# factoryofthesun/distraytracer

Measured on NVIDIA B200. Metric: samples_per_s_1080p_64spp, higher is better.
Workload: dtype f64

## Files before the change

distraytracer_b200/csrc/drt_api.cu:

```cuda
#include <cuda_runtime.h>

#include <algorithm>
#include <cmath>
#include <cstdio>
#include <cstdlib>
#include <cstring>
#include <string>
#include <vector>

#include "../../include/drt.h"
#include "drt_box.cuh"
#include "drt_launch.h"
#include "drt_bvh_order.h"
#include "drt_mesh.h"
#include "drt_skeleton.h"

using namespace drt;

namespace {

thread_local std::string g_err;
int fail(int code, const std::string& m) { g_err = m; return code; }

#define CK(call)                                                                                   \
// ... 569 lines not shown

template <typename R>
void fillParams(Params<R>& P, const drt_scene* s, const DevScene<R>& ds, const drt_settings& st, const CameraD& c, const drt_tile& tile) {
  memset(&P, 0, sizeof(P));
  P.eye = cv<R>(c.eye); P.X = cv<R>(c.X); P.Y = cv<R>(c.Y); P.Z = cv<R>(c.Z);
  for (int i = 0; i < 12; i++) { P.mcam[i] = (R)c.mcam[i]; P.new_mcam[i] = (R)c.new_mcam[i]; P.cloud_mcam[i] = (R)c.cloud_mcam[i]; }
  P.t = c.t; P.b = c.b; P.r = c.r; P.l = c.l;
  P.near_plane = st.near_plane; P.focal_length = st.focal_length; P.aperture = st.aperture;
  P.xRes = st.xRes; P.yRes = st.yRes;
  P.n = (int)sqrt((double)st.antialias_samples);
  P.spp = P.n * P.n;
  P.antialias_samples = st.antialias_samples;
  P.brdf_samples = st.brdf_samples; P.blur_samples = st.blur_samples; P.frame_range = st.frame_range; P.max_depth = st.max_depth;
  P.reflect = st.reflect; P.nogloss = st.nogloss; P.perlin_cloud = st.perlin_cloud; P.cloud_only = st.cloud_only;
  P.frame = st.frame; P.frame_prism = st.frame_prism; P.frame_blur = st.frame_blur; P.frame_cloud = st.frame_cloud;
  P.move_per_frame = st.move_per_frame; P.accel_t = st.accel_t; P.refr_air = st.refr_air; P.refr_glass = st.refr_glass;
  P.phong = st.phong; P.seed = st.seed; P.blur_mode = st.blur_mode;
  P.swept_cull = (st.blur_mode == DRT_BLUR_VELOCITY && st.frame_range <= DRT_SWEPT_FRAMES) ? 1 : 0;
  P.sun = cv<R>(normalized(V(st.sundir)));
  f3(P.sun_outer, st.sun_outer); f3(P.sun_inner, st.sun_inner); f3(P.sun_core, st.sun_core);
  f3(P.bluesky, st.bluesky); f3(P.redsky, st.redsky);
  P.saturation = st.saturation; P.clouddist = st.clouddist; P.cloudhoff = st.cloudhoff;
  P.x0 = tile.x0; P.y0 = tile.y0; P.w = tile.width; P.h = tile.height;
  P.geoms = ds.geoms; P.n_geoms = ds.n_geoms; P.gbounds = ds.gbounds; P.geom_tree = ds.geom_tree >= 0 ? ds.gbounds + ds.geom_tree : nullptr; P.nodes = ds.nodes; P.n_nodes = ds.n_nodes; P.prims = ds.prims; P.lights = ds.lights; P.n_lights = ds.n_lights;
  P.tex = s->d_tex; P.texdims = s->d_texdims;
  if (s->has_mesh) {
    P.mesh_nodes = s->mesh.nodes; P.n_mesh_tris = s->mesh.n_tris; P.mesh_prim = (int)s->prims.size();
    if constexpr (sizeof(R) == 8) P.mesh_tris = s->mesh.tris_f64; else P.mesh_tris = s->mesh.tris_f32;
    P.mesh_mat = s->mesh.mat_ids;
    const drt_prim& m0 = s->mesh_materials[0];
    P.mesh_vel = mk<R>((R)m0.velocity[0], (R)m0.velocity[1], (R)m0.velocity[2]);
  } else P.mesh_vel = mk<R>(R(0), R(0), R(0));
}

int ensureScratch(drt_scene* s, size_t n_samples, size_t n_corners, size_t n_out) {
  CK(s->samples.reserve(n_samples * sizeof(float4)));
  CK(s->need.reserve(n_corners));
  CK(s->bg.reserve(n_corners * sizeof(float4)));
  CK(s->out_u8.reserve(n_out));
  CK(s->out_f32.reserve(n_out * sizeof(float)));
  CK(s->counts.reserve(sizeof(Counts)));
  CK(s->batch_counter.reserve(sizeof(unsigned long long)));
  if (!s->overflow) { CK(s->overflow.reserve(sizeof(int))); CK(cudaMemsetAsync(s->overflow, 0, sizeof(int), s->stream)); }
  return DRT_OK;
}

long long maxChunkSamples() {
// ... 623 lines not shown
```

distraytracer_b200/csrc/drt_device.cuh:

```cuda
#pragma once
#include <cuda_runtime.h>
#include <stdint.h>
#include <float.h>
#include <math.h>
#include <utility>

#include "drt_rng.cuh"

#define DRT_PI 3.14159265358979323846
#define DRT_NODE_STACK 64

namespace drt {

template <typename R> struct Vec { R x, y, z; };

template <typename R> __host__ __device__ inline Vec<R> mk(R x, R y, R z) { Vec<R> v; v.x = x; v.y = y; v.z = z; return v; }
template <typename R> __host__ __device__ inline Vec<R> operator+(Vec<R> a, Vec<R> b) { return mk<R>(a.x + b.x, a.y + b.y, a.z + b.z); }
template <typename R> __host__ __device__ inline Vec<R> operator-(Vec<R> a, Vec<R> b) { return mk<R>(a.x - b.x, a.y - b.y, a.z - b.z); }
template <typename R> __host__ __device__ inline Vec<R> operator-(Vec<R> a) { return mk<R>(-a.x, -a.y, -a.z); }
template <typename R> __host__ __device__ inline Vec<R> operator*(Vec<R> a, R s) { return mk<R>(a.x * s, a.y * s, a.z * s); }
template <typename R> __host__ __device__ inline Vec<R> operator*(R s, Vec<R> a) { return mk<R>(s * a.x, s * a.y, s * a.z); }
template <typename R> __host__ __device__ inline Vec<R> operator/(Vec<R> a, R s) { return mk<R>(a.x / s, a.y / s, a.z / s); }
template <typename R> __host__ __device__ inline R dot(Vec<R> a, Vec<R> b) { return a.x * b.x + (a.y * b.y + a.z * b.z); }
template <typename R> __host__ __device__ inline R norm(Vec<R> a) { return sqrt(dot(a, a)); }
// ... 111 lines not shown
template <typename R>
struct Params {
  Vec<R> eye, X, Y, Z;
  R mcam[12], new_mcam[12], cloud_mcam[12];
  float t, b, r, l;
  float near_plane, focal_length, aperture;
  int xRes, yRes;
  int n, spp, antialias_samples;
  int brdf_samples, blur_samples, frame_range, max_depth;
  int reflect, nogloss, perlin_cloud, cloud_only;
  int frame, frame_prism, frame_blur, frame_cloud;
  int swept_cull;
  float move_per_frame, accel_t, refr_air, refr_glass, phong;
  uint32_t seed;
  int blur_mode;
  Vec<R> sun;
  float sun_outer[3], sun_inner[3], sun_core[3], bluesky[3], redsky[3];
  float saturation, clouddist, cloudhoff;
  int x0, y0, w, h;
  const Geom<R>* geoms; int n_geoms;
  const float4* gbounds;
  const float4* geom_tree;
  const NodeD<R>* nodes; int n_nodes;
  const PrimD<R>* prims;
  const LightD<R>* lights; int n_lights;
  const float4* mesh_nodes; const MeshTri<R>* mesh_tris; int n_mesh_tris; int mesh_prim;
  const unsigned short* mesh_mat;
  Vec<R> mesh_vel;
  const cudaTextureObject_t* tex; const int2* texdims;
  float4* samples;
  unsigned char* need;
  float4* bg;
  float* out_f32;
  unsigned char* out_u8;
  Counts* counts;
  long long sample_base;
  long long sample_count;
  void* pool_raw;
  int pool_cap;
  unsigned long long* batch_counter;
  int unit_samples;
  int steal;
  unsigned char* owned;
  unsigned long long* corner_counter;
  int* overflow;
};

#define SF_ABORT 1u
// ... 32 lines not shown
```

distraytracer_b200/csrc/drt_kernels.cuh:

```cuda
#pragma once
#include "drt_device.cuh"
#include "drt_launch.h"
#include <cstddef>

#ifndef DRT_FORCE_TREE
#define DRT_FORCE_TREE 0
#endif

namespace drt {


template <typename R>
struct alignas(16) Task {
  Vec<R> org, dir;
  float k;
  uint32_t path;
  float dt;
  unsigned char depth;
  unsigned char bits;
  unsigned short slot;
};
#define TASK_CHAIN 1
#define TASK_ROOT 2
static_assert(sizeof(Task<double>) == 64 && sizeof(Task<float>) == 48, "ray records are whole 16-byte words");
// ... 313 lines not shown
  else { if (tmax <= eps || tmin >= t_max) return false; t = tmin; }
  float tmin_tmp = FLT_MAX, t_tmp;
  int last = -1, in_tmp;
  for (int i = 0; i < pr.n_holes; i++) {
    if (inside) { if (holeIntersect<R>(pr.holes[i], ray, start, t_tmp, in_tmp) && t_tmp <= tmin_tmp) { tmin_tmp = t_tmp; last = i; } }
    else if (holeIntersectMax<R>(pr.holes[i], ray, start, t_tmp) && t_tmp < tmin_tmp) { tmin_tmp = t_tmp; last = i; }
  }
  if (last >= 0) {
    const Vec<R> checknorm = prismHolesNorm<R>(pr, ray + (R)t * start, -1, aborted);
    if (aborted) return false;
    const Vec<R> shapenorm = holeNorm<R>(pr.holes[last], ray + (R)tmin_tmp * start);
    if (vecApprox<R>(checknorm, shapenorm) || vecApprox<R>(checknorm, -shapenorm)) return false;
  }
  return true;
}

struct HitRec {
  float t;
  int geom;
  int inside;
  int checker_sel;
};

template <typename R, int F>
__device__ inline bool geomIntersect(const Params<R>& P, const Geom<R>& g, int gi, const int type, const Moved<R>& mv,
                                     const Vec<R>& ray, const Vec<R>& start, float& t_hit, int& inside, int& sel) {
  bool ok = false;
  inside = 0; sel = 0;
    if ((F & FT_BOX) && type == G_BOX) {
      return boxIntersect<R>(P.prims[g.owner], shiftPoint<R, F>(mv, 0, g.vel, g.p0), shiftPoint<R, F>(mv, 0, g.vel, g.p1), ray, start, t_hit, inside, sel);
    } else if (type == G_RECT || type == G_CHECKER) {
      Vec<R> A = shiftPoint<R, F>(mv, g.flags, g.vel, g.p0);
      if (type == G_CHECKER) {
        if (dot(g.p1, ray) == R(0)) return false;
      }
      float c1, c2;
      ok = rectHit<R>(A, g.p1, g.p2, g.p3, g.len1, g.len2, g.eps, ray, start, t_hit, c1, c2);
      if (ok && type == G_CHECKER) {
        if (g.flags & GF_HAS_HOLE) {
          const Geom<R>& hgeo = P.geoms[gi + 1];
          float th, d1, d2;
          if (rectHit<R>(hgeo.p0, hgeo.p1, hgeo.p2, hgeo.p3, hgeo.len1, hgeo.len2, hgeo.eps, ray, start, th, d1, d2))
            ok = false;
        }
        if (ok) {
          int i = (int)(c1 / g.f2);
          int j = (int)(c2 / g.f2);
          int pi = i % 2, pj = j % 2;
          if (pi == 0) { if (pj == 0) sel = 1; if (pj == 1) sel = 2; }
          if (pi == 1) { if (pj == 0) sel = 2; if (pj == 1) sel = 1; }
        }
      }
    } else if (type == G_SPHERE) {
      Vec<R> sc = start - shiftPoint<R, F>(mv, g.flags, g.vel, g.p0);
      float A = (float)dot(ray, ray);
      float B = (float)(R(2) * dot(ray, sc));
      float C = (float)(dot(sc, sc) - (R)((double)g.f0 * (double)g.f0));
      float disc = (float)((double)B * (double)B - (double)(4 * A * C));
      if (disc < 0) return false;
      float sq = sqrtf(disc);
      float t0 = (-B + sq) / (2 * A);
      float t1 = (-B - sq) / (2 * A);
      if (t0 <= 0.001f && t1 <= 0.001f) return false;
// ... 195 lines not shown
    if (!boxHit<R, F>(P.nodes[ni], ray, inv_ray, start, mv)) return false;
  }
  return true;
}

template <typename R, int F, bool COUNT>
__device__ inline void closestHit(const Params<R>& P, const SlabTab gb, const Moved<R>& mv, const Vec<R>& ray,
                                  const Vec<R>& start, HitRec& h, Counts& cnt) {
  h.t = FLT_MAX; h.geom = -1; h.inside = 0; h.checker_sel = 0;
  if ((!(F & FT_REFBLUR) || mv.val == 0.0f) && !DRT_FORCE_TREE) {
    const float ix = 1.0f / (float)ray.x, iy = 1.0f / (float)ray.y, iz = 1.0f / (float)ray.z;
    const float ox = -(float)start.x * ix, oy = -(float)start.y * iy, oz = -(float)start.z * iz;
    const float serr = 4e-7f * (fabsf(ox) + fabsf(oy) + fabsf(oz));
    const bool cull = !((F & FT_VEL) && mv.velocity_mode) || P.swept_cull;
    const bool smem = !(F & FT_BIG) || P.n_geoms <= DRT_SMEM_GEOMS;
    if ((F & FT_BIG) && cull && P.geom_tree) {
      SlabRay st = slabRay(ix, iy, iz, ox, oy, oz, FLT_MAX);
      int2 stack[DRT_NODE_STACK];
      int sp = 0, cur = 0;
      for (;;) {
        while (cur >= 0) { if (COUNT) cnt.node_tests += 4; cur = bvh4Visit<true>(P.geom_tree, cur, st, stack, sp, P.overflow); }
        if (cur == DRT_MESH_DONE) break;
        const int gi = -cur - 1;
        const Geom<R>& g = P.geoms[gi];
        const int type = g.type;
        if (COUNT) cnt.geom_tests[type]++;
        float t_hit; int inside, sel;
        if (geomIntersect<R, F>(P, g, gi, type, mv, ray, start, t_hit, inside, sel) && (t_hit < h.t || (t_hit == h.t && gi < h.geom)) &&
            (!(F & FT_SPILL) || !(g.flags & GF_SPILL) || ((F & FT_VEL) && mv.velocity_mode) || gatherReplay<R, F, COUNT>(P, g.leaf, ray, start, mv, cnt))) {
          h.t = t_hit; h.geom = gi; h.inside = inside; h.checker_sel = sel;
          st.lim = (t_hit * 1.0001f + 1e-4f) + serr;
        }
        cur = bvh4Pop<true>(stack, sp, st.lim);
      }
      return;
    }
    const SlabRay sr = slabRay(ix, iy, iz, ox, oy, oz, FLT_MAX);
    const int n = P.n_geoms;
    for (int g0 = 0; g0 < n; g0 += 32) {
      const int g1 = min(n, g0 + 32);
      unsigned int mask = !cull ? slabAll(g0, g1) : smem ? slabMask<true>(gb, n, g0, g1, sr) : slabMask<false>(gb, n, g0, g1, sr);
      while (mask) {
        const int gi = g0 + __ffs(mask) - 1;
        mask &= mask - 1;
        const Geom<R>& g = P.geoms[gi];
        const int type = g.type;
        if (type == G_HOLE) continue;
        if (cull && h.t < FLT_MAX && !slabMayHit(g.blo, g.bhi, ox, oy, oz, ix, iy, iz, h.t * 1.0001f + 1e-4f, serr)) continue;
        if (COUNT) cnt.geom_tests[type]++;
        float t_hit; int inside, sel;
        if (geomIntersect<R, F>(P, g, gi, type, mv, ray, start, t_hit, inside, sel) && t_hit < h.t &&
            (!(F & FT_SPILL) || !(g.flags & GF_SPILL) || ((F & FT_VEL) && mv.velocity_mode) || gatherReplay<R, F, COUNT>(P, g.leaf, ray, start, mv, cnt))) {
          h.t = t_hit; h.geom = gi; h.inside = inside; h.checker_sel = sel;
        }
      }
    }
    return;
  }
  int stack[DRT_NODE_STACK];
  int sp = 0;
  stack[sp++] = 0;
  const Vec<R> inv_ray = mk<R>(R(1) / ray.x, R(1) / ray.y, R(1) / ray.z);
  while (sp > 0) {
    const NodeD<R>& nd = P.nodes[stack[--sp]];
    if (COUNT) cnt.node_tests++;
    if (!boxHit<R, F>(nd, ray, inv_ray, start, mv)) continue;
    if (!nd.leaf) { stack[sp++] = nd.left; stack[sp++] = nd.right; continue; }
    const int g_end = nd.first + nd.count;
    for (int gi = nd.first; gi < g_end; gi++) {
      const Geom<R>& g = P.geoms[gi];
      const int type = g.type;
      if (type == G_HOLE) continue;
      if (COUNT) cnt.geom_tests[type]++;
      float t_hit; int inside, sel;
      if (geomIntersect<R, F>(P, g, gi, type, mv, ray, start, t_hit, inside, sel) && t_hit < h.t) {
        h.t = t_hit; h.geom = gi; h.inside = inside; h.checker_sel = sel;
      }
    }
  }
}

template <typename R, int F>
__device__ inline bool geomShadow(const Params<R>& P, const Geom<R>& g, int gi, const int type, const Moved<R>& mv,
                                  const Vec<R>& ray, const Vec<R>& start, const float t_max, float& t_occ, bool& aborted) {
    t_occ = 0.0f;
    if ((F & FT_BOX) && type == G_BOX) {
      return boxShadow<R>(P.prims[g.owner], shiftPoint<R, F>(mv, 0, g.vel, g.p0), shiftPoint<R, F>(mv, 0, g.vel, g.p1), ray, start, t_max, aborted);
    } else if (type == G_RECT || type == G_CHECKER) {
      Vec<R> A = shiftPoint<R, F>(mv, g.flags, g.vel, g.p0);
      float eps = (type == G_CHECKER && !(g.flags & GF_HAS_HOLE)) ? 1e-4f : g.eps;
      float th, c1, c2;
      if (rectHit<R>(A, g.p1, g.p2, g.p3, g.len1, g.len2, eps, ray, start, th, c1, c2) && th < t_max) {
        if (g.flags & GF_HAS_HOLE) {
          const Geom<R>& hgeo = P.geoms[gi + 1];
          float t2, d1, d2;
          if (rectHit<R>(hgeo.p0, hgeo.p1, hgeo.p2, hgeo.p3, hgeo.len1, hgeo.len2, hgeo.eps, ray, start, t2, d1, d2) &&
              t2 < t_max)
            return false;
        }
        t_occ = th;
        return true;
      }
    } else if (type == G_SPHERE) {
      const float eps = 1e-3f;
      Vec<R> sc = start - shiftPoint<R, F>(mv, g.flags, g.vel, g.p0);
      float A = (float)dot(ray, ray);
      float B = (float)(R(2) * dot(ray, sc));
      float C = (float)(dot(sc, sc) - (R)((double)g.f0 * (double)g.f0));
      float disc = (float)((double)B * (double)B - (double)(4 * A * C));
      if (disc < 0) return false;
      float sq = sqrtf(disc);
      float t0 = (-B + sq) / (2 * A);
      float t1 = (-B - sq) / (2 * A);
      if ((t0 <= eps || t0 >= t_max) && (t1 <= eps || t1 >= t_max)) return false;
      t_occ = (t0 > eps && t0 < t_max) ? t0 : t1;
      return true;
    } else if (type == G_CYL) {
// ... 31 lines not shown
      if (u < 0 || u > 1) return false;
      Vec<R> DA0 = cross(A0, r1);
      float v = (float)((double)dot(ray, DA0) * (double)invdet);
      if (v < 0 || u + v > 1) return false;
      float t_final = (float)((double)dot(r2, DA0) * (double)invdet);
      if (t_final > 0.001f && t_final < t_max) { t_occ = t_final; return true; }
    }
  return false;
}

template <typename R, int F, bool COUNT>
__device__ inline bool anyHit(const Params<R>& P, const SlabTab gb, const Moved<R>& mv, const Vec<R>& gather_ray,
                              const Vec<R>& gather_start, const Vec<R>& ray, const Vec<R>& start, float t_max, int skip_owner,
                              Counts& cnt, bool& aborted) {
  if ((!(F & FT_REFBLUR) || mv.val == 0.0f) && !DRT_FORCE_TREE) {
    const float ix = 1.0f / (float)ray.x, iy = 1.0f / (float)ray.y, iz = 1.0f / (float)ray.z;
    const float ox = -(float)start.x * ix, oy = -(float)start.y * iy, oz = -(float)start.z * iz;
    const bool cull = !((F & FT_VEL) && mv.velocity_mode) || P.swept_cull;
    const float gather_lead = t_max * 1e-3f;
    const int n = P.n_geoms;
    const bool smem = !(F & FT_BIG) || n <= DRT_SMEM_GEOMS;
    const SlabRay sr = slabRay(ix, iy, iz, ox, oy, oz, t_max * 1.0001f + 1e-4f);
    auto candidate = [&](const int gi) -> int {
      const Geom<R>& g = P.geoms[gi];
      const int type = g.type;
      if (type == G_HOLE || g.owner == skip_owner) return 0;
      if (COUNT) cnt.geom_tests[type]++;
      float t_occ;
      if (!geomShadow<R, F>(P, g, gi, type, mv, ray, start, t_max, t_occ, aborted)) return ((F & FT_BOX) && aborted) ? -1 : 0;
      if ((F & FT_VEL) && mv.velocity_mode) return 1;
      if (t_occ > gather_lead * 1.001f + 2e-3f && !((F & FT_SPILL) && (g.flags & GF_SPILL))) return 1;
      return gatherReplay<R, F, COUNT>(P, g.leaf, gather_ray, gather_start, mv, cnt) ? 1 : 0;
    };
    if ((F & FT_BIG) && cull && P.geom_tree) {
      int2 stack[DRT_NODE_STACK];
      int sp = 0, cur = 0;
      for (;;) {
        while (cur >= 0) { if (COUNT) cnt.node_tests += 4; cur = bvh4Visit<false>(P.geom_tree, cur, sr, stack, sp, P.overflow); }
        if (cur == DRT_MESH_DONE) break;
        if (candidate(-cur - 1) == 1) return true;
        cur = bvh4Pop<false>(stack, sp, sr.lim);
      }
      return false;
    }
    for (int g0 = 0; g0 < n; g0 += 32) {
      const int g1 = min(n, g0 + 32);
      unsigned int mask = !cull ? slabAll(g0, g1) : smem ? slabMask<true>(gb, n, g0, g1, sr) : slabMask<false>(gb, n, g0, g1, sr);
      while (mask) {
        const int gi = g0 + __ffs(mask) - 1;
        mask &= mask - 1;
        const int c = candidate(gi);
        if (c == 1) return true;
        if ((F & FT_BOX) && c == -1) return false;
      }
    }
    return false;
  }
  int stack[DRT_NODE_STACK];
  int sp = 0;
  stack[sp++] = 0;
  const Vec<R> inv_ray = mk<R>(R(1) / gather_ray.x, R(1) / gather_ray.y, R(1) / gather_ray.z);
  while (sp > 0) {
    const NodeD<R>& nd = P.nodes[stack[--sp]];
    if (COUNT) cnt.node_tests++;
    if (!boxHit<R, F>(nd, gather_ray, inv_ray, gather_start, mv)) continue;
    if (!nd.leaf) { stack[sp++] = nd.left; stack[sp++] = nd.right; continue; }
    const int g_end = nd.first + nd.count;
    for (int gi = nd.first; gi < g_end; gi++) {
      const Geom<R>& g = P.geoms[gi];
      const int type = g.type;
      if (type == G_HOLE) continue;
      if (g.owner == skip_owner) continue;
      if (COUNT) cnt.geom_tests[type]++;
      float t_occ;
      if (geomShadow<R, F>(P, g, gi, type, mv, ray, start, t_max, t_occ, aborted)) return true;
      if ((F & FT_BOX) && aborted) return false;
    }
  }
  return false;
}

template <typename R>
__device__ __forceinline__ float meshTriT(const Vec<R>& tA, const Vec<R>& tB, const Vec<R>& tC, const Vec<R>& ray, const Vec<R>& start) {
  const Vec<R> r1 = tB - tA, r2 = tC - tA;
  const Vec<R> hh = cross(ray, r2);
  const float det = (float)dot(r1, hh);
  const float invdet = 1.0f / det;
  if (det >= -0.0001f && det <= 0.0001f) return -1.f;
  const Vec<R> A0 = start - tA;
  const float u = (float)((double)invdet * (double)dot(A0, hh));
  if (u < 0 || u > 1) return -1.f;
  const Vec<R> DA0 = cross(A0, r1);
// ... 158 lines not shown
  int inside_sel;
  int slot;
};

template <typename R>
__device__ __forceinline__ int meshOwner(const Params<R>& P, const int tri) {
  return P.mesh_prim + (P.mesh_mat ? (int)__ldg(P.mesh_mat + tri) : 0);
}

template <typename R, int F, bool COUNT>
__device__ inline bool traceRay(const Params<R>& P, const SlabTab gb, const Task<R>& T, HitRec& h, int& motion,
                                Counts& cnt) {
  motion = -1;
  if (T.depth == 0) return false;
  if (COUNT) cnt.rays++;
  const Moved<R> mv = makeMoved<R, F>(P, T.dt);
  closestHit<R, F, COUNT>(P, gb, mv, T.dir, T.org, h, cnt);
  if ((F & FT_MESH) && P.n_mesh_tris > 0) {
    meshTraverse<R, F, COUNT, true>(P, T.dir, T.org, h.t, &h, T.dir, T.org, (F & FT_VEL) && mv.velocity_mode, mv.time, cnt);
  }
  if ((F & (FT_VEL | FT_REFBLUR)) && (T.bits & TASK_CHAIN)) motion = 0;
  if (h.geom < 0) return false;
  if ((F & (FT_VEL | FT_REFBLUR)) && (T.bits & TASK_CHAIN)) {
    const int owner = h.geom >= P.n_geoms ? meshOwner(P, h.geom - P.n_geoms) : P.geoms[h.geom].owner;
    motion = (P.prims[owner].flags & 2) ? 1 : 0;
  }
  return true;
}

template <typename R>
struct ShadeState {
  Vec<R> isectP, normal, e;
  Moved<R> mv;
  float shape_color[3];
  float k;
  uint32_t path;
  int prim;
  int tri;
  bool lights;
  bool aborted, early;
  int hits;
  double tmp[3];
};

template <typename R>
struct PairIn {
  Vec<R> isectP;
  uint32_t path;
  float val, dt;
  int want;
};
template <typename R>
struct PairOut {
  R* x; R* y; R* z;
  unsigned char* state;
};
template <typename R>
__host__ __device__ constexpr size_t pairOutBytes() { return (size_t)32 * DRT_PAIR_LIGHTS * 3 * sizeof(R); }

template <typename R, int F, bool COUNT>
__device__ void shadeA(const Params<R>& P, const Task<R>& T, const HitRec& h, Task<R>* stack, int& n_out, double (&add)[3],
                       bool& has_add, bool& aborted, ShadeState<R>& S, Counts& cnt) {
  int sp = 0;
  n_out = 0; has_add = false;
  add[0] = add[1] = add[2] = 0.0;
  const Moved<R> mv = makeMoved<R, F>(P, T.dt);
  S.lights = false; S.aborted = false; S.early = false; S.hits = 0; S.tmp[0] = S.tmp[1] = S.tmp[2] = 0.0; S.mv = mv;
  do {
    const Vec<R> ray = T.dir, eye = T.org;
    const float k = T.k;
    const int mesh_tri = ((F & FT_MESH) && h.geom >= P.n_geoms) ? h.geom - P.n_geoms : -1;
    const int owner = mesh_tri >= 0 ? meshOwner(P, mesh_tri) : P.geoms[h.geom].owner;
    const PrimD<R>& pr = P.prims[owner];

    const Vec<R> isectP = eye + (R)h.t * ray;
    Vec<R> normal;
    if (pr.type == 0) {
      Vec<R> nn = isectP - shiftPoint<R, F>(mv, 0, pr.vel, pr.pA);
      normal = nn / norm(nn);
    } else if (pr.type == 1 || pr.type == 7) {
      const Vec<R> c1 = shiftPoint<R, F>(mv, 0, pr.vel, pr.pA);
      Vec<R> axis = pr.pG;
      if ((F & FT_VEL) && (pr.flags & 64) && mv.velocity_mode) axis = normalized((pr.n1 + pr.n2 * mv.time) - c1);
      Vec<R> pc = isectP - c1;
      normal = normalized(pc - dot(pc, axis) * axis);
    } else if ((F & FT_BOX) && pr.type == 9) {
      const float eps = 1e-3f;
      const Vec<R> pa = isectP - shiftPoint<R, F>(mv, 0, pr.vel, pr.pA);
      if (dot(pa, pr.n0) <= (R)eps) normal = pr.n0;
      else if (dot(pa, pr.n1) <= (R)eps) normal = pr.n1;
      else if (dot(pa, pr.n2) <= (R)eps) normal = pr.n2;
      else { aborted = true; break; }
    } else if ((F & FT_BOX) && pr.type == 10) {
      normal = prismHolesNorm<R>(pr, isectP, h.checker_sel >= 3 ? h.checker_sel - 3 : -1, aborted);
      if (aborted) break;
    } else if (pr.type == 4 || ((F & FT_BOX) && pr.type == 8)) {
// ... 134 lines not shown
        for (int c = 0; c < 3; c++) add[c] += ((double)k * (double)shape_color[c]) * f;
        has_add = true;
      }
      if (pr.name == 3) {
        float dist = (float)((double)(norm(isectP - pr.eA) + norm(isectP - pr.eB) + norm(isectP - pr.eC) + norm(isectP - pr.eD)) /
                             (double)pr.e_den);
        double f = 0.1 * (double)dist + 0.05 * pow5((double)dist) + 0.9;
        for (int c = 0; c < 3; c++) add[c] += ((double)k * (double)shape_color[c]) * f;
        has_add = true;
      }
      continue;
    }

    S.isectP = isectP; S.normal = normal; S.e = normalized(eye - isectP);
    S.shape_color[0] = shape_color[0]; S.shape_color[1] = shape_color[1]; S.shape_color[2] = shape_color[2];
    S.k = k; S.path = T.path; S.prim = owner; S.tri = mesh_tri; S.lights = true;
  } while (0);
  n_out = sp;
}

template <typename R, int F, bool COUNT>
__device__ void shadowPair(const Params<R>& P, const SlabTab gb, const PairIn<R>& in, int li, const PairOut<R>& out, const int oi,
                           Counts& cnt) {
  const LightD<R>& L = P.lights[li];
  const Vec<R> isectP = in.isectP;
  Moved<R> mv;
  mv.val = (F & FT_REFBLUR) ? in.val : 0.0f;
  mv.time = (F & FT_VEL) ? (R)in.dt : R(0);
  mv.velocity_mode = (F & FT_VEL) ? ((((F & FT_REFBLUR) ? P.blur_mode == 1 : true) && in.dt != 0.0f) ? 1 : 0) : 0;
  Vec<R> sray;
  if (L.type == 0) sray = L.center - isectP;
  else if (L.type == 2) sray = rectSample<R>(L.A, L.B, L.D, in.path, rng_dim_light(li, 0)) - isectP;
  else {
    if (!sampleSphereLight<R>(L, isectP, in.path, li, sray)) { out.state[oi] = 2; return; }
    out.x[oi] = sray.x; out.y[oi] = sray.y; out.z[oi] = sray.z;
  }
  const float t_max = (float)norm(sray);
  const Vec<R> sdir = normalized(sray);
  if (COUNT) cnt.shadow_rays++;
  bool threw = false;
  bool occluded = anyHit<R, F, COUNT>(P, gb, mv, sray, isectP + sray * R(1e-3), sdir, isectP + sdir * R(1e-3), t_max, L.prim_index, cnt, threw);
  if ((F & FT_BOX) && threw) { out.state[oi] = 2; return; }
  if ((F & FT_MESH) && !occluded && P.n_mesh_tris > 0)
    occluded = meshTraverse<R, F, COUNT, false>(P, sdir, isectP + sdir * R(1e-3), t_max, nullptr, sray, isectP + sray * R(1e-3),
                                                (F & FT_VEL) && mv.velocity_mode, mv.time, cnt);
  out.state[oi] = occluded ? 0 : 1;
}

template <typename R, int F, bool COUNT>
__device__ void shadeB(const Params<R>& P, ShadeState<R>& S, const PairOut<R>& res, const int hit_lane, int l0, int l1, Counts& cnt) {
  const PrimD<R>& pr = P.prims[S.prim];
  for (int li = l0; li < l1 && !S.early && !S.aborted; li++) {
    const int oi = (li - l0) * 32 + hit_lane;
    const int state = res.state[oi];
    if (state == 2) { S.aborted = true; break; }
    if (state == 0) continue;
    const LightD<R>& L = P.lights[li];
    Vec<R> sray;
    if (L.type == 0) sray = L.center - S.isectP;
    else if (L.type == 2) sray = rectSample<R>(L.A, L.B, L.D, S.path, rng_dim_light(li, 0)) - S.isectP;
    else sray = mk<R>(res.x[oi], res.y[oi], res.z[oi]);
    const Vec<R> sdir = normalized(sray);
      if ((F & FT_TEX) && (pr.flags & 4)) {
        float u = 0, v = 0; int type = 0;
        if (pr.type == 3 || pr.type == 5 || pr.type == 4) {
          Vec<R> uA = shiftPoint<R, F>(S.mv, pr.name == 1 ? GF_NAME_RECTANGLE : 0, pr.vel, pr.uvA);
          Vec<R> uD = shiftPoint<R, F>(S.mv, pr.name == 1 ? GF_NAME_RECTANGLE : 0, pr.vel, pr.uvD);
          u = (float)(norm(cross(S.isectP - uA, pr.uv_ad)) / pr.uv_den_u);
          v = (float)(norm(cross(S.isectP - uD, pr.uv_dc)) / pr.uv_den_v);
          type = 1;
        } else if ((F & FT_BOX) && pr.type >= 8 && pr.type <= 10) {
          const Vec<R> uA = shiftPoint<R, F>(S.mv, 0, pr.vel, pr.uvA), uD = shiftPoint<R, F>(S.mv, 0, pr.vel, pr.uvD);
          if (fabs(dot(cross(pr.uv_ad, pr.uv_dc), S.isectP)) <= R(1e-5)) {
            u = (float)(norm(cross(S.isectP - uA, pr.uv_ad)) / pr.uv_den_u);
            v = (float)(norm(cross(S.isectP - uD, pr.uv_dc)) / pr.uv_den_v);
            type = 1;
          } else type = 0;
        } else if (pr.type == 6) {
          Vec<R> V_hit = S.isectP - pr.rA;
          float check1 = (float)dot(pr.re1, V_hit), check2 = (float)dot(pr.re2, V_hit);
// ... 134 lines not shown
    const uint32_t li = (uint32_t)(perm ? lensIndexFromTable(perm + (pt - perm_pt0) * P.antialias_samples, s, P.antialias_samples)
                                        : lensIndexScan(pkey, s, P.antialias_samples));
    float r = (float)((double)(P.aperture / 2) * (double)rng_u01(pkey, 4u * li));
    float theta = (float)(2 * DRT_PI * (double)rng_u01(pkey, 4u * li + 1));
    double snd, csd;
    sincos((double)theta, &snd, &csd);
    const float cs = (float)csd, sn = (float)snd;
    eye_sample = P.eye + (R)(r * cs) * P.X + (R)(r * sn) * P.Y;
  }
  const int ii = s / P.n, jj = s % P.n;
  float adj_x = (float)((double)x + ((double)(float)ii + (double)rng_u01(pkey, 4u * s + 2)) / 9.0);
  float adj_y = (float)((double)y + ((double)(float)jj + (double)rng_u01(pkey, 4u * s + 3)) / 9.0);
  pi = (int)(double)adj_x; pj = (int)(double)adj_y;
  const Vec<R> rayDir = eyeRay<R>(P, pi, pj);
  const Vec<R> focalPoint = P.eye + (R)P.focal_length * rayDir;
  org = eye_sample;
  dir = focalPoint - eye_sample;
}

#ifndef DRT_WAVE_CTAS_PER_SM
#define DRT_WAVE_CTAS_PER_SM 1
#endif
#define DRT_HIT_BUCKETS 64
__host__ __device__ constexpr size_t waveDynSmemBytes() { return (size_t)DRT_CTA_SLOTS * 28 + (size_t)DRT_CTA_HITS * 3; }
template <typename R>
__host__ __device__ constexpr size_t waveScratchBytes(int pool_cap) {
  return (size_t)pool_cap * sizeof(Task<R>) + DRT_CTA_HITS * sizeof(HitRef) + DRT_WAVE_WARPS * pairOutBytes<R>() +
         3 * (size_t)(pool_cap / 32) * sizeof(uint32_t);
}

template <typename R, int F, bool COUNT>
__global__ void __launch_bounds__(32 * DRT_WAVE_WARPS, DRT_WAVE_CTAS_PER_SM) render_wave(const __grid_constant__ Params<R> P) {
  extern __shared__ __align__(16) unsigned char s_dyn[];
  unsigned long long(*s_acc)[3] = (unsigned long long(*)[3])s_dyn;
  unsigned int* s_flags = (unsigned int*)(s_dyn + (size_t)DRT_CTA_SLOTS * 24);
  unsigned short* s_order = (unsigned short*)(s_dyn + (size_t)DRT_CTA_SLOTS * 28);
  unsigned char* s_hkey = s_dyn + (size_t)DRT_CTA_SLOTS * 28 + (size_t)DRT_CTA_HITS * 2;
  __shared__ int s_nst, s_nfree, s_ninfl, s_npush, s_count, s_nhits, s_grab, s_state, s_nvalid;
  __shared__ int s_hist[DRT_HIT_BUCKETS];
  __shared__ long long s_idx0, s_unit_next, s_unit_end;
  __shared__ float4 s_gb[3 * DRT_SMEM_GEOMS / 2 + 2 * DRT_SMEM_GEOMS / 8];
  SlabTab gb; gb.g = P.gbounds; gb.s = 0u;
  if (!(F & FT_BIG) || P.n_geoms <= DRT_SMEM_GEOMS) {
    for (int i = threadIdx.x; i < slabPairWords(P.n_geoms) + 2 * ((P.n_geoms + 7) / 8); i += blockDim.x) s_gb[i] = P.gbounds[i];
    gb.s = (unsigned)__cvta_generic_to_shared(s_gb);
  }
  const unsigned FULL = 0xffffffffu;
  const int lane = threadIdx.x & 31, wib = threadIdx.x >> 5, tid = threadIdx.x;
  const size_t cap = (size_t)P.pool_cap;
  const int n_chunks = P.pool_cap >> 5;
  char* cbase = (char*)P.pool_raw + (size_t)blockIdx.x * waveScratchBytes<R>(P.pool_cap);
  uint4* pool = (uint4*)cbase;
  uint4* hits = (uint4*)(cbase + cap * sizeof(Task<R>));
  char* wbase = (char*)(hits + DRT_CTA_HITS) + (size_t)wib * pairOutBytes<R>();
  uint32_t* stk = (uint32_t*)((char*)(hits + DRT_CTA_HITS) + (size_t)DRT_WAVE_WARPS * pairOutBytes<R>());
  uint32_t* fre = stk + n_chunks;
  uint32_t* infl = fre + n_chunks;
  PairOut<R> pairout;
  __shared__ unsigned char s_pstate[DRT_WAVE_WARPS * 32 * DRT_PAIR_LIGHTS];
  pairout.x = (R*)wbase; pairout.y = pairout.x + 32 * DRT_PAIR_LIGHTS; pairout.z = pairout.y + 32 * DRT_PAIR_LIGHTS;
  pairout.state = s_pstate + wib * 32 * DRT_PAIR_LIGHTS;
  unsigned long long(*acc)[3] = s_acc;
  unsigned int* sfl = s_flags;
  const long long n_units = (P.sample_count + P.unit_samples - 1) / P.unit_samples;

  Counts cnt;
  if (COUNT) { cnt.samples = 0; cnt.rays = 0; cnt.shadow_rays = 0; cnt.shade_evals = 0; cnt.noise_evals = 0; cnt.node_tests = 0;
               for (int i = 0; i < 7; i++) cnt.geom_tests[i] = 0; }
// ... 513 lines not shown
```

distraytracer_b200/csrc/drt_launch.h:

```cpp
#pragma once
#include "drt_device.cuh"

#ifndef DRT_WAVE_WARPS
#define DRT_WAVE_WARPS 16
#endif
#ifndef DRT_BATCH
#define DRT_BATCH 64
#endif
#define DRT_CTA_SLOTS (DRT_WAVE_WARPS * DRT_BATCH)
#ifndef DRT_TRACE_HITS_TARGET
#define DRT_TRACE_HITS_TARGET 8192
#endif
#define DRT_HITS_PER_PASS (DRT_TRACE_HITS_TARGET + 32 * DRT_WAVE_WARPS)
#define DRT_CTA_HITS (DRT_HITS_PER_PASS + 64)
#define DRT_MAX_CHILDREN 6
#ifndef DRT_PAIR_LIGHTS
#define DRT_PAIR_LIGHTS 8
#endif
#define DRT_SMEM_GEOMS 256

enum WaveFeat {
  FT_MESH = 1,
  FT_VEL = 2,
  FT_REFBLUR = 4,
  FT_GLASS = 8,
  FT_TEX = 16,
  FT_BIG = 32,
  FT_BOX = 64,
  FT_SPILL = 128,
  FT_ALL = 255
};

#define DRT_WAVE_FEATS {FT_GLASS | FT_TEX, 0, FT_TEX, FT_VEL, FT_MESH | FT_TEX, FT_MESH | FT_VEL | FT_TEX, FT_REFBLUR | FT_GLASS | FT_TEX, FT_ALL}

namespace drt {
const int* waveFeatList(int* n);
int waveFeatPick(int need);
template <typename R> int waveGridBlocks();
template <typename R> size_t wavePoolBytes(int blocks, int pool_cap);
template <typename R> int launchRenderSamples(const Params<R>& P, bool collect, int feat, int blocks, cudaStream_t q);
template <typename R> using WaveFnT = void (*)(Params<R>);
template <typename R, int GROUP> WaveFnT<R> waveKernelOfGroup(int feat, bool collect);
template <typename R> void launchCloudCorners(const Params<R>& P, cudaStream_t q);
template <typename R> void launchResolve(const Params<R>& P, int row0, int rows, cudaStream_t q);
void launchNeedPush(const unsigned char* mine, unsigned char* shared, size_t n, cudaStream_t q);
}
```

distraytracer_b200/csrc/drt_launch_impl.cuh:

```cuda
#include <algorithm>
#include "drt_kernels.cuh"
#include "drt_launch.h"

namespace drt {
typedef WaveFnT<DRT_REAL> WaveFn;
#define DRT_WAVE_CASE(mask) if (feat == (mask) && !collect) return render_wave<DRT_REAL, (mask), false>
#if DRT_GROUP == 0
template <> WaveFn waveKernelOfGroup<DRT_REAL, 0>(int feat, bool collect) {
  DRT_WAVE_CASE(FT_GLASS | FT_TEX);
  DRT_WAVE_CASE(0);
  DRT_WAVE_CASE(FT_TEX);
  return nullptr;
}
#elif DRT_GROUP == 1
template <> WaveFn waveKernelOfGroup<DRT_REAL, 1>(int feat, bool collect) {
  DRT_WAVE_CASE(FT_VEL);
  DRT_WAVE_CASE(FT_MESH | FT_TEX);
  DRT_WAVE_CASE(FT_MESH | FT_VEL | FT_TEX);
  return nullptr;
}
#else
template <> WaveFn waveKernelOfGroup<DRT_REAL, 2>(int feat, bool collect) {
  DRT_WAVE_CASE(FT_REFBLUR | FT_GLASS | FT_TEX);
  DRT_WAVE_CASE(FT_ALL);
  if (feat == FT_ALL && collect) return render_wave<DRT_REAL, FT_ALL, true>;
  return nullptr;
}
#endif

#if DRT_GROUP == 0
static WaveFn waveKernel(int feat, bool collect) {
  WaveFn f = waveKernelOfGroup<DRT_REAL, 0>(feat, collect);
  if (!f) f = waveKernelOfGroup<DRT_REAL, 1>(feat, collect);
  if (!f) f = waveKernelOfGroup<DRT_REAL, 2>(feat, collect);
  return f;
}
template <> int waveGridBlocks<DRT_REAL>() {
  int dev = 0, sms = 0, per_sm = 1 << 30, n = 0;
  cudaGetDevice(&dev);
  cudaDeviceGetAttribute(&sms, cudaDevAttrMultiProcessorCount, dev);
  const int* list = waveFeatList(&n);
  for (int i = 0; i <= n; i++) {
    WaveFn f = i < n ? waveKernel(list[i], false) : waveKernel(FT_ALL, true);
    int k = 0;
    cudaFuncSetAttribute((const void*)f, cudaFuncAttributeMaxDynamicSharedMemorySize, (int)waveDynSmemBytes());
    cudaOccupancyMaxActiveBlocksPerMultiprocessor(&k, (const void*)f, 32 * DRT_WAVE_WARPS, waveDynSmemBytes());
    per_sm = k < per_sm ? k : per_sm;
  }
  if (per_sm < 1) per_sm = 1;
  return sms * per_sm;
}
template <> size_t wavePoolBytes<DRT_REAL>(int blocks, int pool_cap) { return (size_t)blocks * waveScratchBytes<DRT_REAL>(pool_cap); }
template <> int launchRenderSamples<DRT_REAL>(const Params<DRT_REAL>& P, bool collect, int feat, int blocks, cudaStream_t q) {
  const int pick = collect ? FT_ALL : waveFeatPick(feat);
  waveKernel(pick, collect)<<<blocks, 32 * DRT_WAVE_WARPS, waveDynSmemBytes(), q>>>(P);
  return pick;
}
template <> void launchCloudCorners<DRT_REAL>(const Params<DRT_REAL>& P, cudaStream_t q) {
  const int n = (P.w + 1) * (P.h + 1);
  int blocks = (n + DRT_CLOUD_BLOCK - 1) / DRT_CLOUD_BLOCK;
  if (P.corner_counter) {
    int dev = 0, sms = 0;
    cudaGetDevice(&dev);
    cudaDeviceGetAttribute(&sms, cudaDevAttrMultiProcessorCount, dev);
    blocks = std::min(blocks, sms * 16);
  }
  cloud_corners<DRT_REAL><<<blocks, 128, 0, q>>>(P);
}
#ifdef DRT_DEFINE_SHARED_LAUNCHERS
void launchNeedPush(const unsigned char* mine, unsigned char* shared, size_t n, cudaStream_t q) {
  need_push<<<(unsigned)((n + 255) / 256), 256, 0, q>>>(mine, shared, n);
}
#endif
template <> void launchResolve<DRT_REAL>(const Params<DRT_REAL>& P, int row0, int rows, cudaStream_t q) {
  resolve<DRT_REAL><<<(P.w * rows + 255) / 256, 256, 0, q>>>(P, row0, rows);
}
#endif
}
// ... 1 lines not shown
```

Baseline: 776.8.

## Stage geometry, primitive and light records in shared memory per CTA

Adds an FT_RECS kernel variant that copies the Geom, PrimD and LightD arrays into dynamic shared memory at CTA start when the scene is small enough, then routes all record lookups through accessor functions. The goal is to replace repeated global/L1 loads of scene records during traversal and shading with shared-memory reads. It doubles the number of kernel instantiations, adds extra dynamic shared memory per block that could lower occupancy, and adds a startup copy to each CTA.

```diff
diff --git a/distraytracer_b200/csrc/drt_api.cu b/distraytracer_b200/csrc/drt_api.cu
--- a/distraytracer_b200/csrc/drt_api.cu
+++ b/distraytracer_b200/csrc/drt_api.cu
@@ -615,7 +615,9 @@
   f3(P.bluesky, st.bluesky); f3(P.redsky, st.redsky);
   P.saturation = st.saturation; P.clouddist = st.clouddist; P.cloudhoff = st.cloudhoff;
   P.x0 = tile.x0; P.y0 = tile.y0; P.w = tile.width; P.h = tile.height;
-  P.geoms = ds.geoms; P.n_geoms = ds.n_geoms; P.gbounds = ds.gbounds; P.geom_tree = ds.geom_tree >= 0 ? ds.gbounds + ds.geom_tree : nullptr; P.nodes = ds.nodes; P.n_nodes = ds.n_nodes; P.prims = ds.prims; P.lights = ds.lights; P.n_lights = ds.n_lights;
+  P.geoms = ds.geoms; P.n_geoms = ds.n_geoms; P.gbounds = ds.gbounds; P.geom_tree = ds.geom_tree >= 0 ? ds.gbounds + ds.geom_tree : nullptr; P.nodes = ds.nodes; P.n_nodes = ds.n_nodes; P.prims = ds.prims; P.n_prims = ds.n_prims; P.lights = ds.lights; P.n_lights = ds.n_lights;
+  const size_t recs = sizeof(Geom<R>) * ds.n_geoms + sizeof(PrimD<R>) * ds.n_prims + sizeof(LightD<R>) * ds.n_lights;
+  P.smem_recs = (ds.n_geoms <= DRT_SMEM_GEOMS && recs <= DRT_SMEM_RECS) ? (int)recs : 0;
   P.tex = s->d_tex; P.texdims = s->d_texdims;
   if (s->has_mesh) {
     P.mesh_nodes = s->mesh.nodes; P.n_mesh_tris = s->mesh.n_tris; P.mesh_prim = (int)s->prims.size();
diff --git a/distraytracer_b200/csrc/drt_device.cuh b/distraytracer_b200/csrc/drt_device.cuh
--- a/distraytracer_b200/csrc/drt_device.cuh
+++ b/distraytracer_b200/csrc/drt_device.cuh
@@ -157,8 +157,9 @@
   const float4* gbounds;
   const float4* geom_tree;
   const NodeD<R>* nodes; int n_nodes;
-  const PrimD<R>* prims;
+  const PrimD<R>* prims; int n_prims;
   const LightD<R>* lights; int n_lights;
+  int smem_recs;
   const float4* mesh_nodes; const MeshTri<R>* mesh_tris; int n_mesh_tris; int mesh_prim;
   const unsigned short* mesh_mat;
   Vec<R> mesh_vel;
diff --git a/distraytracer_b200/csrc/drt_kernels.cuh b/distraytracer_b200/csrc/drt_kernels.cuh
--- a/distraytracer_b200/csrc/drt_kernels.cuh
+++ b/distraytracer_b200/csrc/drt_kernels.cuh
@@ -359,13 +359,33 @@
   int checker_sel;
 };
 
+extern __shared__ __align__(16) unsigned char s_dyn[];
+__host__ __device__ constexpr size_t waveDynSmemBytes() { return (size_t)DRT_CTA_SLOTS * 28 + (size_t)DRT_CTA_HITS * 3; }
+static_assert(waveDynSmemBytes() % 16 == 0, "the staged records start on a 16-byte boundary");
+
+template <typename R, int F>
+__device__ __forceinline__ const Geom<R>* geomRecs(const Params<R>& P) {
+  return (F & FT_RECS) ? (const Geom<R>*)(s_dyn + waveDynSmemBytes()) : P.geoms;
+}
+template <typename R, int F>
+__device__ __forceinline__ const PrimD<R>* primRecs(const Params<R>& P) {
+  return (F & FT_RECS) ? (const PrimD<R>*)(geomRecs<R, F>(P) + P.n_geoms) : P.prims;
+}
+template <typename R, int F>
+__device__ __forceinline__ const LightD<R>* lightRecs(const Params<R>& P) {
+  return (F & FT_RECS) ? (const LightD<R>*)(primRecs<R, F>(P) + P.n_prims) : P.lights;
+}
+__device__ __forceinline__ void ctaCopy16(void* dst, const void* src, const int bytes) {
+  for (int i = threadIdx.x; i < bytes / 16; i += blockDim.x) ((uint4*)dst)[i] = __ldg((const uint4*)src + i);
+}
+
 template <typename R, int F>
 __device__ inline bool geomIntersect(const Params<R>& P, const Geom<R>& g, int gi, const int type, const Moved<R>& mv,
                                      const Vec<R>& ray, const Vec<R>& start, float& t_hit, int& inside, int& sel) {
   bool ok = false;
   inside = 0; sel = 0;
     if ((F & FT_BOX) && type == G_BOX) {
-      return boxIntersect<R>(P.prims[g.owner], shiftPoint<R, F>(mv, 0, g.vel, g.p0), shiftPoint<R, F>(mv, 0, g.vel, g.p1), ray, start, t_hit, inside, sel);
+      return boxIntersect<R>(primRecs<R, F>(P)[g.owner], shiftPoint<R, F>(mv, 0, g.vel, g.p0), shiftPoint<R, F>(mv, 0, g.vel, g.p1), ray, start, t_hit, inside, sel);
     } else if (type == G_RECT || type == G_CHECKER) {
       Vec<R> A = shiftPoint<R, F>(mv, g.flags, g.vel, g.p0);
       if (type == G_CHECKER) {
@@ -375,7 +395,7 @@
       ok = rectHit<R>(A, g.p1, g.p2, g.p3, g.len1, g.len2, g.eps, ray, start, t_hit, c1, c2);
       if (ok && type == G_CHECKER) {
         if (g.flags & GF_HAS_HOLE) {
-          const Geom<R>& hgeo = P.geoms[gi + 1];
+          const Geom<R>& hgeo = geomRecs<R, F>(P)[gi + 1];
           float th, d1, d2;
           if (rectHit<R>(hgeo.p0, hgeo.p1, hgeo.p2, hgeo.p3, hgeo.len1, hgeo.len2, hgeo.eps, ray, start, th, d1, d2))
             ok = false;
@@ -617,7 +637,7 @@
         while (cur >= 0) { if (COUNT) cnt.node_tests += 4; cur = bvh4Visit<true>(P.geom_tree, cur, st, stack, sp, P.overflow); }
         if (cur == DRT_MESH_DONE) break;
         const int gi = -cur - 1;
-        const Geom<R>& g = P.geoms[gi];
+        const Geom<R>& g = geomRecs<R, F>(P)[gi];
         const int type = g.type;
         if (COUNT) cnt.geom_tests[type]++;
         float t_hit; int inside, sel;
@@ -638,7 +658,7 @@
       while (mask) {
         const int gi = g0 + __ffs(mask) - 1;
         mask &= mask - 1;
-        const Geom<R>& g = P.geoms[gi];
+        const Geom<R>& g = geomRecs<R, F>(P)[gi];
         const int type = g.type;
         if (type == G_HOLE) continue;
         if (cull && h.t < FLT_MAX && !slabMayHit(g.blo, g.bhi, ox, oy, oz, ix, iy, iz, h.t * 1.0001f + 1e-4f, serr)) continue;
@@ -663,7 +683,7 @@
     if (!nd.leaf) { stack[sp++] = nd.left; stack[sp++] = nd.right; continue; }
     const int g_end = nd.first + nd.count;
     for (int gi = nd.first; gi < g_end; gi++) {
-      const Geom<R>& g = P.geoms[gi];
+      const Geom<R>& g = geomRecs<R, F>(P)[gi];
       const int type = g.type;
       if (type == G_HOLE) continue;
       if (COUNT) cnt.geom_tests[type]++;
@@ -680,14 +700,14 @@
                                   const Vec<R>& ray, const Vec<R>& start, const float t_max, float& t_occ, bool& aborted) {
     t_occ = 0.0f;
     if ((F & FT_BOX) && type == G_BOX) {
-      return boxShadow<R>(P.prims[g.owner], shiftPoint<R, F>(mv, 0, g.vel, g.p0), shiftPoint<R, F>(mv, 0, g.vel, g.p1), ray, start, t_max, aborted);
+      return boxShadow<R>(primRecs<R, F>(P)[g.owner], shiftPoint<R, F>(mv, 0, g.vel, g.p0), shiftPoint<R, F>(mv, 0, g.vel, g.p1), ray, start, t_max, aborted);
     } else if (type == G_RECT || type == G_CHECKER) {
       Vec<R> A = shiftPoint<R, F>(mv, g.flags, g.vel, g.p0);
       float eps = (type == G_CHECKER && !(g.flags & GF_HAS_HOLE)) ? 1e-4f : g.eps;
       float th, c1, c2;
       if (rectHit<R>(A, g.p1, g.p2, g.p3, g.len1, g.len2, eps, ray, start, th, c1, c2) && th < t_max) {
         if (g.flags & GF_HAS_HOLE) {
-          const Geom<R>& hgeo = P.geoms[gi + 1];
+          const Geom<R>& hgeo = geomRecs<R, F>(P)[gi + 1];
           float t2, d1, d2;
           if (rectHit<R>(hgeo.p0, hgeo.p1, hgeo.p2, hgeo.p3, hgeo.len1, hgeo.len2, hgeo.eps, ray, start, t2, d1, d2) &&
               t2 < t_max)
@@ -765,7 +785,7 @@
     const bool smem = !(F & FT_BIG) || n <= DRT_SMEM_GEOMS;
     const SlabRay sr = slabRay(ix, iy, iz, ox, oy, oz, t_max * 1.0001f + 1e-4f);
     auto candidate = [&](const int gi) -> int {
-      const Geom<R>& g = P.geoms[gi];
+      const Geom<R>& g = geomRecs<R, F>(P)[gi];
       const int type = g.type;
       if (type == G_HOLE || g.owner == skip_owner) return 0;
       if (COUNT) cnt.geom_tests[type]++;
@@ -810,7 +830,7 @@
     if (!nd.leaf) { stack[sp++] = nd.left; stack[sp++] = nd.right; continue; }
     const int g_end = nd.first + nd.count;
     for (int gi = nd.first; gi < g_end; gi++) {
-      const Geom<R>& g = P.geoms[gi];
+      const Geom<R>& g = geomRecs<R, F>(P)[gi];
       const int type = g.type;
       if (type == G_HOLE) continue;
       if (g.owner == skip_owner) continue;
@@ -1015,8 +1035,8 @@
   if ((F & (FT_VEL | FT_REFBLUR)) && (T.bits & TASK_CHAIN)) motion = 0;
   if (h.geom < 0) return false;
   if ((F & (FT_VEL | FT_REFBLUR)) && (T.bits & TASK_CHAIN)) {
-    const int owner = h.geom >= P.n_geoms ? meshOwner(P, h.geom - P.n_geoms) : P.geoms[h.geom].owner;
-    motion = (P.prims[owner].flags & 2) ? 1 : 0;
+    const int owner = h.geom >= P.n_geoms ? meshOwner(P, h.geom - P.n_geoms) : geomRecs<R, F>(P)[h.geom].owner;
+    motion = (primRecs<R, F>(P)[owner].flags & 2) ? 1 : 0;
   }
   return true;
 }
@@ -1063,8 +1083,8 @@
     const Vec<R> ray = T.dir, eye = T.org;
     const float k = T.k;
     const int mesh_tri = ((F & FT_MESH) && h.geom >= P.n_geoms) ? h.geom - P.n_geoms : -1;
-    const int owner = mesh_tri >= 0 ? meshOwner(P, mesh_tri) : P.geoms[h.geom].owner;
-    const PrimD<R>& pr = P.prims[owner];
+    const int owner = mesh_tri >= 0 ? meshOwner(P, mesh_tri) : geomRecs<R, F>(P)[h.geom].owner;
+    const PrimD<R>& pr = primRecs<R, F>(P)[owner];
 
     const Vec<R> isectP = eye + (R)h.t * ray;
     Vec<R> normal;
@@ -1245,7 +1265,7 @@
 template <typename R, int F, bool COUNT>
 __device__ void shadowPair(const Params<R>& P, const SlabTab gb, const PairIn<R>& in, int li, const PairOut<R>& out, const int oi,
                            Counts& cnt) {
-  const LightD<R>& L = P.lights[li];
+  const LightD<R>& L = lightRecs<R, F>(P)[li];
   const Vec<R> isectP = in.isectP;
   Moved<R> mv;
   mv.val = (F & FT_REFBLUR) ? in.val : 0.0f;
@@ -1272,13 +1292,13 @@
 
 template <typename R, int F, bool COUNT>
 __device__ void shadeB(const Params<R>& P, ShadeState<R>& S, const PairOut<R>& res, const int hit_lane, int l0, int l1, Counts& cnt) {
-  const PrimD<R>& pr = P.prims[S.prim];
+  const PrimD<R>& pr = primRecs<R, F>(P)[S.prim];
   for (int li = l0; li < l1 && !S.early && !S.aborted; li++) {
     const int oi = (li - l0) * 32 + hit_lane;
     const int state = res.state[oi];
     if (state == 2) { S.aborted = true; break; }
     if (state == 0) continue;
-    const LightD<R>& L = P.lights[li];
+    const LightD<R>& L = lightRecs<R, F>(P)[li];
     Vec<R> sray;
     if (L.type == 0) sray = L.center - S.isectP;
     else if (L.type == 2) sray = rectSample<R>(L.A, L.B, L.D, S.path, rng_dim_light(li, 0)) - S.isectP;
@@ -1459,7 +1479,6 @@
 #define DRT_WAVE_CTAS_PER_SM 1
 #endif
 #define DRT_HIT_BUCKETS 64
-__host__ __device__ constexpr size_t waveDynSmemBytes() { return (size_t)DRT_CTA_SLOTS * 28 + (size_t)DRT_CTA_HITS * 3; }
 template <typename R>
 __host__ __device__ constexpr size_t waveScratchBytes(int pool_cap) {
   return (size_t)pool_cap * sizeof(Task<R>) + DRT_CTA_HITS * sizeof(HitRef) + DRT_WAVE_WARPS * pairOutBytes<R>() +
@@ -1468,7 +1487,6 @@
 
 template <typename R, int F, bool COUNT>
 __global__ void __launch_bounds__(32 * DRT_WAVE_WARPS, DRT_WAVE_CTAS_PER_SM) render_wave(const __grid_constant__ Params<R> P) {
-  extern __shared__ __align__(16) unsigned char s_dyn[];
   unsigned long long(*s_acc)[3] = (unsigned long long(*)[3])s_dyn;
   unsigned int* s_flags = (unsigned int*)(s_dyn + (size_t)DRT_CTA_SLOTS * 24);
   unsigned short* s_order = (unsigned short*)(s_dyn + (size_t)DRT_CTA_SLOTS * 28);
@@ -1481,6 +1499,11 @@
   if (!(F & FT_BIG) || P.n_geoms <= DRT_SMEM_GEOMS) {
     for (int i = threadIdx.x; i < slabPairWords(P.n_geoms) + 2 * ((P.n_geoms + 7) / 8); i += blockDim.x) s_gb[i] = P.gbounds[i];
     gb.s = (unsigned)__cvta_generic_to_shared(s_gb);
+  }
+  if (F & FT_RECS) {
+    ctaCopy16((void*)geomRecs<R, F>(P), P.geoms, P.n_geoms * (int)sizeof(Geom<R>));
+    ctaCopy16((void*)primRecs<R, F>(P), P.prims, P.n_prims * (int)sizeof(PrimD<R>));
+    ctaCopy16((void*)lightRecs<R, F>(P), P.lights, P.n_lights * (int)sizeof(LightD<R>));
   }
   const unsigned FULL = 0xffffffffu;
   const int lane = threadIdx.x & 31, wib = threadIdx.x >> 5, tid = threadIdx.x;
diff --git a/distraytracer_b200/csrc/drt_launch.h b/distraytracer_b200/csrc/drt_launch.h
--- a/distraytracer_b200/csrc/drt_launch.h
+++ b/distraytracer_b200/csrc/drt_launch.h
@@ -18,6 +18,7 @@
 #define DRT_PAIR_LIGHTS 8
 #endif
 #define DRT_SMEM_GEOMS 256
+#define DRT_SMEM_RECS (32 * 1024)
 
 enum WaveFeat {
   FT_MESH = 1,
@@ -28,7 +29,8 @@
   FT_BIG = 32,
   FT_BOX = 64,
   FT_SPILL = 128,
-  FT_ALL = 255
+  FT_ALL = 255,
+  FT_RECS = 256
 };
 
 #define DRT_WAVE_FEATS {FT_GLASS | FT_TEX, 0, FT_TEX, FT_VEL, FT_MESH | FT_TEX, FT_MESH | FT_VEL | FT_TEX, FT_REFBLUR | FT_GLASS | FT_TEX, FT_ALL}
diff --git a/distraytracer_b200/csrc/drt_launch_impl.cuh b/distraytracer_b200/csrc/drt_launch_impl.cuh
--- a/distraytracer_b200/csrc/drt_launch_impl.cuh
+++ b/distraytracer_b200/csrc/drt_launch_impl.cuh
@@ -4,7 +4,9 @@
 
 namespace drt {
 typedef WaveFnT<DRT_REAL> WaveFn;
-#define DRT_WAVE_CASE(mask) if (feat == (mask) && !collect) return render_wave<DRT_REAL, (mask), false>
+#define DRT_WAVE_CASE(mask)                                                                                              \
+  if ((feat & ~FT_RECS) == (mask) && !collect)                                                                           \
+    return (feat & FT_RECS) ? render_wave<DRT_REAL, (mask) | FT_RECS, false> : render_wave<DRT_REAL, (mask), false>
 #if DRT_GROUP == 0
 template <> WaveFn waveKernelOfGroup<DRT_REAL, 0>(int feat, bool collect) {
   DRT_WAVE_CASE(FT_GLASS | FT_TEX);
@@ -22,8 +24,7 @@
 #else
 template <> WaveFn waveKernelOfGroup<DRT_REAL, 2>(int feat, bool collect) {
   DRT_WAVE_CASE(FT_REFBLUR | FT_GLASS | FT_TEX);
-  DRT_WAVE_CASE(FT_ALL);
-  if (feat == FT_ALL && collect) return render_wave<DRT_REAL, FT_ALL, true>;
+  if (feat == FT_ALL) return collect ? render_wave<DRT_REAL, FT_ALL, true> : render_wave<DRT_REAL, FT_ALL, false>;
   return nullptr;
 }
 #endif
@@ -40,20 +41,25 @@
   cudaGetDevice(&dev);
   cudaDeviceGetAttribute(&sms, cudaDevAttrMultiProcessorCount, dev);
   const int* list = waveFeatList(&n);
-  for (int i = 0; i <= n; i++) {
-    WaveFn f = i < n ? waveKernel(list[i], false) : waveKernel(FT_ALL, true);
+  auto fit = [&](WaveFn f, const size_t smem) {
     int k = 0;
-    cudaFuncSetAttribute((const void*)f, cudaFuncAttributeMaxDynamicSharedMemorySize, (int)waveDynSmemBytes());
-    cudaOccupancyMaxActiveBlocksPerMultiprocessor(&k, (const void*)f, 32 * DRT_WAVE_WARPS, waveDynSmemBytes());
+    cudaFuncSetAttribute((const void*)f, cudaFuncAttributeMaxDynamicSharedMemorySize, (int)smem);
+    cudaOccupancyMaxActiveBlocksPerMultiprocessor(&k, (const void*)f, 32 * DRT_WAVE_WARPS, smem);
     per_sm = k < per_sm ? k : per_sm;
+  };
+  for (int i = 0; i < n; i++) {
+    fit(waveKernel(list[i], false), waveDynSmemBytes());
+    if (list[i] != FT_ALL) fit(waveKernel(list[i] | FT_RECS, false), waveDynSmemBytes() + DRT_SMEM_RECS);
   }
+  fit(waveKernel(FT_ALL, true), waveDynSmemBytes());
   if (per_sm < 1) per_sm = 1;
   return sms * per_sm;
 }
 template <> size_t wavePoolBytes<DRT_REAL>(int blocks, int pool_cap) { return (size_t)blocks * waveScratchBytes<DRT_REAL>(pool_cap); }
 template <> int launchRenderSamples<DRT_REAL>(const Params<DRT_REAL>& P, bool collect, int feat, int blocks, cudaStream_t q) {
-  const int pick = collect ? FT_ALL : waveFeatPick(feat);
-  waveKernel(pick, collect)<<<blocks, 32 * DRT_WAVE_WARPS, waveDynSmemBytes(), q>>>(P);
+  int pick = collect ? FT_ALL : waveFeatPick(feat);
+  if (pick != FT_ALL && P.smem_recs) pick |= FT_RECS;
+  waveKernel(pick, collect)<<<blocks, 32 * DRT_WAVE_WARPS, waveDynSmemBytes() + ((pick & FT_RECS) ? P.smem_recs : 0), q>>>(P);
   return pick;
 }
 template <> void launchCloudCorners<DRT_REAL>(const Params<DRT_REAL>& P, cudaStream_t q) {
```

Result: faster. 813.5, median of 6 (+4.7%).
